# PM25/Information-Retrieval-with-Contrastive-Learning

Hardware: AMD Instinct MI355X
Metric: query-doc pairs/sec (train) + queries/sec @ top-k over N docs, 1/2/4/8 GPU (higher is better)
Workload: dtype bf16

## Files before the change

include/irc.h:

```cpp
#ifndef IRC_H_
#define IRC_H_

#include <stdint.h>

#ifdef __cplusplus
extern "C" {
#endif

typedef void* irc_stream_t;

#define IRC_OK 0
#define IRC_E_INVALID 1001
#define IRC_E_WORKSPACE 1002
#define IRC_E_LAUNCH 1003

const char* irc_last_error(void);
int irc_abi_version(void);

int64_t irc_scan_topk_workspace(int64_t Q, int64_t N, int64_t D, int64_t k);
int irc_scan_topk(const void* queries, const void* docs, int64_t Q, int64_t N, int64_t D,
                  int64_t k, int64_t doc_offset, void* workspace, int64_t workspace_bytes,
                  float* out_score, int64_t* out_idx, irc_stream_t stream);

int irc_scan_topk_many(const void* const* queries, int64_t batches, const void* docs, int64_t Q,
// ... 57 lines not shown
                      int64_t workspace_bytes, float* out_score, int64_t* out_idx,
                      irc_stream_t stream);
int irc_scan_scores_fp8(const void* queries, const void* docs, int64_t Q, int64_t N, int64_t D,
                        float* out, irc_stream_t stream);
int irc_quantize_fp8(int in_dtype, const void* x, int64_t n, float scale, void* out,
                     irc_stream_t stream);

int irc_gemm(int in_dtype, int out_dtype, int a_layout, int b_layout, int epilogue, int64_t M,
             int64_t N, int64_t K, float alpha, const void* A, int64_t lda, int64_t strideA,
             const void* B, int64_t ldb, int64_t strideB, const float* bias, int64_t strideBias,
             const void* R, int64_t ldr, int64_t strideR, void* C, int64_t ldc, int64_t strideC,
             int accumulate, int64_t batch, void* workspace, int64_t workspace_bytes,
             irc_stream_t stream);
int64_t irc_gemm_workspace(int in_dtype, int out_dtype, int epilogue, int64_t M, int64_t N,
                           int64_t K, int64_t batch);
int irc_gemm_ex(int in_dtype, int out_dtype, int a_layout, int b_layout, int epilogue, int64_t M,
                int64_t N, int64_t K, float alpha, const void* A, int64_t lda, int64_t strideA,
                const void* B, int64_t ldb, int64_t strideB, const float* bias, int64_t strideBias,
                const void* R, int64_t ldr, int64_t strideR, void* C, int64_t ldc, int64_t strideC,
                int accumulate, int64_t batch, void* workspace, int64_t workspace_bytes,
                int64_t max_blocks, irc_stream_t stream);
int64_t irc_gemm_workspace_ex(int in_dtype, int out_dtype, int epilogue, int64_t M, int64_t N,
                              int64_t K, int64_t batch, int64_t max_blocks);
int irc_gemm_set_persistent(int mode);
int irc_gemm_set_big_ring(int on);
int irc_gemm_ln(int epilogue, int64_t M, int64_t N, int64_t K, const void* A, int64_t lda,
                const void* B, int64_t ldb, const float* bias, const void* R, int64_t ldr,
                void* C, int64_t ldc, const float* ln_stats, int ln_nt, const float* ln_gamma,
                const float* ln_beta, float ln_eps, int64_t ln_h, const float* fold_colsum,
                float* stats_out, int* stats_nt_out, irc_stream_t stream);
int irc_gemm_set_big_mf16(int on);
int irc_gemm_set_big_dma(int on);
int irc_gemm_big_dma_fits(int64_t M, int64_t N, int64_t K, int64_t lda, int64_t ldb);

int irc_gemm_set_pp(int on);

int irc_embed_ln(int dtype, const int64_t* ids, const void* word, const void* pos,
                 const void* type0, const float* gamma, const float* beta, void* y, int64_t rows,
                 int64_t L, int64_t H, float eps, irc_stream_t stream);
int irc_layernorm(int dtype, const void* x, void* y, const float* gamma, const float* beta,
                  int64_t rows, int64_t H, float eps, irc_stream_t stream);
int irc_attention(int dtype, const void* qkv, const int64_t* mask, void* ctx, int64_t B,
                  int64_t L, int64_t H, int64_t heads, irc_stream_t stream);
int irc_qkv_attention(int64_t M, int64_t H, int64_t heads, int64_t L, const void* x, int64_t ldx,
                      const void* wqkv_perm, const float* bias_perm, const int64_t* mask,
                      void* ctx, int64_t ldc, irc_stream_t stream);

int64_t irc_layernorm_bwd_workspace(int64_t rows, int64_t H);
int irc_layernorm_bwd(int dtype, int dy_dtype, const void* dy, const void* x, const float* gamma,
                      void* dx, float* dgamma, float* dbeta, float* partial,
                      int64_t partial_floats, int64_t rows, int64_t H, float eps, int64_t bcast_L,
                      float dy_scale, int accumulate, irc_stream_t stream);
int irc_attention_bwd(int dtype, const void* qkv, const int64_t* mask, const void* ctx,
                      const void* dctx, void* dqkv, int64_t B, int64_t L, int64_t H,
                      int64_t heads, irc_stream_t stream);
int irc_embed_sum(int dtype, const int64_t* ids, const void* word, const void* pos,
                  const void* type0, float* y, int64_t rows, int64_t L, int64_t H,
                  irc_stream_t stream);
int irc_embed_bwd(int dtype, const void* dx, const int64_t* ids, float* dword, float* dpos,
                  float* dtype0, float* workspace, int64_t ws_floats, int64_t B, int64_t L,
                  int64_t H, int64_t pad_id, irc_stream_t stream);

int irc_lstm_fwd(int dtype, const float* xp, const void* whh, void* hout, float* gsave,
                 float* csave, void* hprev, int64_t B, int64_t L, int64_t H, int64_t ndir,
                 irc_stream_t stream);
int irc_lstm_bwd(int dtype, const float* dy, const void* whh, const float* gsave,
// ... 159 lines not shown
```

information-retrieval-with-contrastive-learning_amd/csrc/gemm.hip:

```cpp
#include "gemm_epi.h"
#include "gemm_pp.h"

#include <algorithm>
#include <atomic>
#include <type_traits>

#ifndef IRC_GEMM_GROUP_M
#define IRC_GEMM_GROUP_M 0
#endif

namespace irc {
namespace gemm {

enum Layout { ROW = 0, COL = 1 };

constexpr int BM = 128, BN = 128, NT = 256;

template <typename T>
struct TT;
template <>
struct TT<unsigned short> {
  static constexpr int BK = 32;
  static constexpr int VEC = 8;
  static constexpr int PITCH = BK * 2 + 16;
};
template <>
struct TT<float> {
  static constexpr int BK = 16;
  static constexpr int VEC = 4;
  static constexpr int PITCH = BK * 4 + 16;
};

struct Args {
  const void* A;
  const void* B;
  void* C;
  const float* bias;
  const void* R;
  int M, N, K;
  int64_t lda, ldb, ldc, ldr;
  int64_t sA, sB, sC, sR, sBias;
  float alpha;
  int accumulate;
  int vec_a, vec_b;
  int vec_c;
  int kchunk;
  float* P;
  int group_m;
  LnArgs ln;
  int big_dma;
};

__device__ __forceinline__ int kimg_off(int row, int ch) {
  return 256 * row + 16 * (ch ^ (((row & 3) << 2) | ((row >> 2) & 3)));
}
__device__ __forceinline__ bf16x8 kimg_frag(const char* img, int col0, int ks, int lane) {
  const int g = lane >> 4, j = lane & 15, q = j >> 2, p = j & 3;
  const int c = col0 + 16 * (g & 1);
  const int k0 = ks * 16 + 8 * (g >> 1);
  const int cb = c / 8 + (p >> 1), b8 = 8 * (p & 1);
  const v4s lo = ds_tr16(img + kimg_off(k0 + q, cb) + b8);
  const v4s hi = ds_tr16(img + kimg_off(k0 + 4 + q, cb) + b8);
  const v4s both[2] = {lo, hi};
  return __builtin_bit_cast(bf16x8, both);
}

template <typename T, int LAYOUT>
struct Slab {
  static constexpr int BK = TT<T>::BK;
  static constexpr int VEC = TT<T>::VEC;
  static constexpr int NVEC = (128 * BK) / VEC;
  static constexpr int PER_T = NVEC / NT;
  u16x8 v[PER_T];

  __device__ __forceinline__ void load(const T* base, int64_t ld, int row0, int nrows, int k0,
                                       int K, bool vec) {
    const int tid = threadIdx.x;
#pragma unroll
    for (int i = 0; i < PER_T; ++i) {
      const int e = i * NT + tid;
      int r, kk;
      if (LAYOUT == ROW) {
        r = e / (BK / VEC);
// ... 277 lines not shown
template <int ROWS>
__device__ __forceinline__ void stage(const unsigned short* __restrict__ X, int64_t ld, int r0,
                                      int nrows, int k0, char* lds_tile, int wave, int lane,
                                      int ls = 0, int sh = 6) {
  constexpr int PASSES = ROWS * 8 / NT;
#pragma unroll
  for (int i = 0; i < PASSES; ++i) {
    const int p = (i * NW + wave) * 64 + lane;
    const int row = p >> 3;
    const int c = (p & 7) ^ chunk_key(row);
    int gr = ls == 0 ? r0 + row
                     : ((r0 + row) >> sh) * ls + min(row & ((1 << sh) - 1), ls - 1);
    gr = gr < nrows ? gr : nrows - 1;
    glds16(X + (int64_t)gr * ld + k0 + c * 8, lds_tile + (i * NW + wave) * 1024);
  }
}
template <int ROWS>
__device__ __forceinline__ void stage_buf(__amdgpu_buffer_rsrc_t rsrc, uint32_t lane_off,
                                          uint32_t soff, uint32_t pass_bytes, char* lds_tile,
                                          int wave) {
  constexpr int PASSES = ROWS * 8 / NT;
#pragma unroll
  for (int i = 0; i < PASSES; ++i)
    blds16(rsrc, lane_off, soff + i * pass_bytes, lds_tile + (i * NW + wave) * 1024);
}
__device__ __forceinline__ uint32_t dma_lane_off(int64_t ld, int wave, int lane, int ls = 0) {
  const int row0 = 8 * wave + (lane >> 3);
  const int gr = ls == 0 ? row0 : min(row0, ls - 1);
  return (uint32_t)gr * (uint32_t)ld * 2u + (uint32_t)(((lane & 7) ^ chunk_key(row0)) * 16);
}
inline bool dma_fits(int64_t rows, int64_t K, int64_t ld) {
  if (rows <= 0 || K <= 0 || ld < 0 || ld > (1ll << 31)) return false;
  return ((rows - 1) * ld + K) * 2 < (1ll << 31);
}

constexpr int BK4 = 32, ROW4 = BK4 * 2, NST = 4;
template <int ROWS>
__device__ __forceinline__ void stage4(const unsigned short* __restrict__ X, int64_t ld, int r0,
                                       int nrows, int k0, char* lds_tile, int wave, int lane) {
  constexpr int CH = ROWS * 4;
  static_assert(CH % NT == 0, "whole passes");
#pragma unroll
  for (int i = 0; i < CH / NT; ++i) {
    const int p = (i * NW + wave) * 64 + lane;
    const int row = p >> 2;
    const int c = (p & 3) ^ ((row >> 2) & 3);
    int gr = r0 + row;
    gr = gr < nrows ? gr : nrows - 1;
    glds16(X + (int64_t)gr * ld + k0 + c * 8, lds_tile + (i * NW + wave) * 1024);
  }
}

#ifdef IRC_BIG_STAMPS
__device__ uint64_t big_stamps[64][5][2];
#define BSTAMP(kt, i)                                                                      \
  do {                                                                                     \
    __builtin_amdgcn_sched_barrier(0);                                                     \
    if (blockIdx.x == 0 && threadIdx.x == 0 && (kt) < 64) {                               \
      uint64_t c_, r_;                                                                     \
      asm volatile("s_memtime %0\n\ts_memrealtime %1\n\ts_waitcnt lgkmcnt(0)"            \
                   : "=s"(c_), "=s"(r_)::"memory");                                        \
      *(volatile uint64_t*)&big_stamps[(kt)][(i)][0] = c_;                                 \
      *(volatile uint64_t*)&big_stamps[(kt)][(i)][1] = r_;                                 \
    }                                                                                      \
    __builtin_amdgcn_sched_barrier(0);                                                     \
  } while (0)
#else
#define BSTAMP(kt, i) \
  do {                \
  } while (0)
#endif

template <int WNB>
__device__ __forceinline__ void mainloop_mf16(const unsigned short* A, int64_t lda,
                                              const unsigned short* B, int64_t ldb, int m0,
                                              int n0, int M, int N, int K, char* lds, int wave,
                                              int lane, f32x4 (&acc4)[8][2 * WNB], bool dma,
                                              int ls = 0, int sh = 6) {
  constexpr int BN = 128 * WNB;
  constexpr int A_BYTES = BM * ROW_BYTES, STAGE = A_BYTES + BN * ROW_BYTES;
  const int wm = wave >> 2, wn = wave & 3;
  const int nk = K / BK;
  const int a_rows = ls == 0 ? 64 : ls;
  const int a_row0 = ls == 0 ? m0 : (m0 >> sh) * ls;
  const bool buf = dma && (ls == 0 || sh == 6) && a_row0 + (BM / 64) * a_rows <= M && n0 + BN <= N;
  const __amdgpu_buffer_rsrc_t ra = buffer_rsrc(A, (uint32_t)(((int64_t)(M - 1) * lda + K) * 2));
  const __amdgpu_buffer_rsrc_t rb = buffer_rsrc(B, (uint32_t)(((int64_t)(N - 1) * ldb + K) * 2));
  const uint32_t a_pass = (uint32_t)a_rows * (uint32_t)lda * 2u, b_pass = 128u * (uint32_t)ldb;
  const uint32_t a_tile = (uint32_t)a_row0 * (uint32_t)lda * 2u;
  const uint32_t b_tile = (uint32_t)n0 * (uint32_t)ldb * 2u;
  uint32_t a_lane = 0, b_lane = 0;
  if (buf) {
    a_lane = dma_lane_off(lda, wave, lane, ls);
    b_lane = dma_lane_off(ldb, wave, lane);
    stage_buf<BM>(ra, a_lane, a_tile, a_pass, lds, wave);
    stage_buf<BN>(rb, b_lane, b_tile, b_pass, lds + A_BYTES, wave);
  } else {
    stage<BM>(A, lda, m0, M, 0, lds, wave, lane, ls, sh);
    stage<BN>(B, ldb, n0, N, 0, lds + A_BYTES, wave, lane);
  }
  wait_vmcnt<0>();
  __syncthreads();
  const int l16 = lane & 15, q4 = lane >> 4;
  const int key = chunk_key(l16);
  for (int kt = 0; kt < nk; ++kt) {
    const int cur = kt & 1;
#ifdef IRC_PP_DIAG_NODMA
    const bool more = kt + 1 < nk && kt < 0;
#else
    const bool more = kt + 1 < nk;
#endif
    BSTAMP(kt, 0);
    char* nxt = lds + (cur ^ 1) * STAGE;
    if (more && buf) {
      const uint32_t kb = (uint32_t)(kt + 1) * ROW_BYTES;
      stage_buf<BM>(ra, a_lane, a_tile + kb, a_pass, nxt, wave);
      stage_buf<BN>(rb, b_lane, b_tile + kb, b_pass, nxt + A_BYTES, wave);
    } else if (more) {
      int ln = lane;
      asm volatile("" : "+v"(ln));
      stage<BM>(A, lda, m0, M, (kt + 1) * BK, nxt, wave, ln, ls, sh);
      stage<BN>(B, ldb, n0, N, (kt + 1) * BK, nxt + A_BYTES, wave, ln);
    }
    BSTAMP(kt, 1);
    const char* la = lds + cur * STAGE;
    const char* lb = la + A_BYTES;
#pragma unroll
    for (int s2 = 0; s2 < 2; ++s2) {
      const int coff = (((4 * s2 + q4) ^ key) * 16);
      bf16x8 fa[8];
#pragma unroll
      for (int i = 0; i < 8; ++i)
        fa[i] = *reinterpret_cast<const bf16x8*>(la + (wm * 128 + i * 16 + l16) * 128 + coff);
#pragma unroll
      for (int j = 0; j < 2 * WNB; ++j) {
        const bf16x8 fb =
            *reinterpret_cast<const bf16x8*>(lb + (wn * 32 * WNB + j * 16 + l16) * 128 + coff);
#pragma unroll
        for (int i = 0; i < 8; ++i)
          acc4[i][j] = __builtin_amdgcn_mfma_f32_16x16x32_bf16(fa[i], fb, acc4[i][j], 0, 0, 0);
      }
    }
    BSTAMP(kt, 2);
    wait_vmcnt<0>();
    BSTAMP(kt, 3);
    __syncthreads();
    BSTAMP(kt, 4);
  }
}
}

inline std::atomic<int>& big_ring_mode() {
  static std::atomic<int> on{0};
  return on;
}
inline bool big_ring() { return big_ring_mode().load(std::memory_order_relaxed) != 0; }

inline std::atomic<int>& big_mf16_mode() {
  static std::atomic<int> on{1};
  return on;
}
inline bool big_mf16() { return big_mf16_mode().load(std::memory_order_relaxed) != 0; }

inline std::atomic<int>& big_dma_mode() {
  static std::atomic<int> on{1};
  return on;
}
inline int big_dma_flag(int64_t M, int64_t N, int64_t K, int64_t lda, int64_t ldb) {
  return big_dma_mode().load(std::memory_order_relaxed) != 0 && big::dma_fits(M, K, lda) &&
         big::dma_fits(N, K, ldb);
}

template <int EPI, int WNB>
__device__ __forceinline__ void big_epilogue_bf16(const Args& g, const f32x4 (&acc4)[8][2 * WNB],
                                                  char* lds, unsigned short* C,
                                                  const unsigned short* R, const float* bias,
                                                  int m0, int n0, int wave, int lane) {
  constexpr int BN = 128 * WNB, WCOLS = 32 * WNB, PITCH = WCOLS + 8;
  constexpr int CPR = WCOLS / 8;
  constexpr int NCH = 32 * CPR / 64;
  constexpr int NB = CPR == 12 ? 3 : 1;
  constexpr int RSTEP = 64 * NB / CPR;
  static_assert(64 * NB % CPR == 0 && NCH % NB == 0, "the chunk map repeats every NB iterations");
  constexpr bool READS_R = EPI == EPI_BIAS_RESID || EPI == EPI_RESID || EPI == EPI_DGELU;
  constexpr bool USES_R = READS_R || EPI == EPI_BIAS_GELU_SAVE;
  const int wm = wave >> 2, wn = wave & 3;
  float* st = reinterpret_cast<float*>(lds) + wave * (32 * PITCH);
  const int rbase0 = m0 + wm * 128;
  const int cbase = n0 + wn * WCOLS;
  const bool fast = m0 + big::BM <= g.M && n0 + BN <= g.N && g.ldc < (1 << 24) &&
                    (!USES_R || g.ldr < (1 << 24));
  float bv[2 * WNB];
#pragma unroll
  for (int j = 0; j < 2 * WNB; ++j) {
    const int col = cbase + j * 16 + (lane & 15);
    bv[j] = epi_has_bias(EPI) && col < g.N ? bias[col] : 0.f;
  }
  const f32x2_t alpha = {g.alpha, g.alpha};
  float* sw = st + 4 * (lane >> 4) * PITCH + (lane & 15);

  auto finish = [&](const f32x4& v0, const f32x4& v1, const u16x8& rr,
                    const unsigned short* rp) -> u16x8 {
    float v[8] = {v0[0], v0[1], v0[2], v0[3], v1[0], v1[1], v1[2], v1[3]};
// ... 171 lines not shown
    for (int kt = 0; kt < nk; ++kt) {
      const int after = nk - 1 - kt;
      if (after >= 2) wait_vmcnt<2 * PPT>();
      else if (after == 1) wait_vmcnt<PPT>();
      else wait_vmcnt<0>();
      wg_barrier();
      if (kt + 3 < nk) {
        char* nxt = lds + ((kt + 3) & 3) * STG4;
        big::stage4<BM>(A, g.lda, m0, g.M, (kt + 3) * BK4, nxt, wave, lane);
        big::stage4<BN>(B, g.ldb, n0, g.N, (kt + 3) * BK4, nxt + A4, wave, lane);
      }
      const char* la = lds + (kt & 3) * STG4;
      const char* lb = la + A4;
#pragma unroll
      for (int kk = 0; kk < BK4 / 16; ++kk) {
        const int coff = ((2 * kk + h) ^ sw4) * 16;
        bf16x8 fa[4], fb[WNB];
#pragma unroll
        for (int i = 0; i < 4; ++i)
          fa[i] = *reinterpret_cast<const bf16x8*>(la + (wm * 128 + i * 32 + r32) * ROW4 + coff);
#pragma unroll
        for (int j = 0; j < WNB; ++j)
          fb[j] = *reinterpret_cast<const bf16x8*>(lb + (wn * 32 * WNB + j * 32 + r32) * ROW4 + coff);
#pragma unroll
        for (int i = 0; i < 4; ++i)
#pragma unroll
          for (int j = 0; j < WNB; ++j)
            acc[i][j] = __builtin_amdgcn_mfma_f32_32x32x16_bf16(fa[i], fb[j], acc[i][j], 0, 0, 0);
      }
    }
    __syncthreads();
  } else if constexpr (MF16) {
    big::mainloop_mf16<WNB>(A, g.lda, B, g.ldb, m0, n0, g.M, g.N, g.K, lds, wave, lane, acc4,
                            g.big_dma != 0);
  } else {
  const int nk = g.K / BK;
  big::stage<BM>(A, g.lda, m0, g.M, 0, lds, wave, lane);
  big::stage<BN>(B, g.ldb, n0, g.N, 0, lds + A_BYTES, wave, lane);
  wait_vmcnt<0>();
  __syncthreads();
  const int swz = big::chunk_key(r32);
  for (int kt = 0; kt < nk; ++kt) {
    const int cur = kt & 1;
#ifdef IRC_PP_DIAG_NODMA
    const bool more = kt + 1 < nk && kt < 0;
#else
    const bool more = kt + 1 < nk;
#endif
    if (more) {
      char* nxt = lds + (cur ^ 1) * STAGE;
      big::stage<BM>(A, g.lda, m0, g.M, (kt + 1) * BK, nxt, wave, lane);
      big::stage<BN>(B, g.ldb, n0, g.N, (kt + 1) * BK, nxt + A_BYTES, wave, lane);
    }
    const char* la = lds + cur * STAGE;
    const char* lb = la + A_BYTES;
#pragma unroll
    for (int kk = 0; kk < BK / 16; ++kk) {
      const int coff = (((2 * kk + h) ^ swz) * 16);
      bf16x8 fa[4], fb[WNB];
#pragma unroll
      for (int i = 0; i < 4; ++i)
        fa[i] = *reinterpret_cast<const bf16x8*>(la + (wm * 128 + i * 32 + r32) * 128 + coff);
#pragma unroll
      for (int j = 0; j < WNB; ++j)
        fb[j] = *reinterpret_cast<const bf16x8*>(lb + (wn * 32 * WNB + j * 32 + r32) * 128 + coff);
#pragma unroll
      for (int i = 0; i < 4; ++i)
// ... 238 lines not shown
          if constexpr (sizeof(TO) == 2)
            r = bf16_to_f32(reinterpret_cast<const unsigned short*>(R)[(int64_t)row * g.ldr + col]);
          else
            r = reinterpret_cast<const float*>(R)[(int64_t)row * g.ldr + col];
          v = EPI == EPI_DGELU ? v * gelu_grad_fast(r) : v + r;
        }
        TO* dst = C + (int64_t)row * g.ldc + col;
        if constexpr (sizeof(TO) == 2) {
          *reinterpret_cast<unsigned short*>(dst) = f32_to_bf16(v);
        } else {
          if (g.accumulate)
            *reinterpret_cast<float*>(dst) += v;
          else
            *reinterpret_cast<float*>(dst) = v;
        }
      }
    }
  }
}

typedef __bf16 bf16x2_v __attribute__((ext_vector_type(2)));
struct QaArgs {
  const unsigned short* x;
  const unsigned short* w;
  const float* bias;
  const int64_t* mask;
  unsigned short* ctx;
  int M, K, H;
  int64_t ldx, ldc;
  float scale;
  int L;
  int group_m;
  int big_dma;
};

template <int SL>
__global__ __launch_bounds__(big::NT, 1) void qkv_attn_kernel(QaArgs g) {
  constexpr bool PACK = SL == 0;
  constexpr int WNB = 3, BM = big::BM, BN = 128 * WNB, TP = BN + 8;
  constexpr int SLX = PACK ? 128 : SL;
  constexpr int SH = SLX == 64 ? 6 : 7;
  constexpr int NJM = SLX / 32;
  __shared__ __attribute__((aligned(1024))) char lds[2 * (BM + BN) * big::ROW_BYTES];
  static_assert(128 * TP * 2 + 8 * SLX * 4 <= 2 * (BM + BN) * big::ROW_BYTES,
                "staged half and mask biases fit the LDS");
  const int nseq = g.M / g.L;
  const int spt = PACK ? BM / g.L : BM / SLX;
  const int ls = PACK || g.L == SL ? 0 : g.L;
  const int tiles_m = (nseq + spt - 1) / spt;
  const int tiles_n = 3 * g.H / BN;
  const int ntiles = tiles_m * tiles_n;
  int bid = blockIdx.x;
  {
    const int q = ntiles / 8, r = ntiles % 8, x = bid % 8;
    bid = (x < r ? x * (q + 1) : r * (q + 1) + (x - r) * q) + bid / 8;
  }
  int tm, tn;
  grouped_tile(bid, tiles_m, tiles_n, g.group_m, tm, tn);
  const int m0 = PACK ? tm * spt * g.L : tm * BM, n0 = tn * BN;
  const int lane = threadIdx.x & 63;
  const int wave = __builtin_amdgcn_readfirstlane(threadIdx.x >> 6);
  const int wm = wave >> 2, wn = wave & 3;
  f32x4 acc4[8][2 * WNB];
#pragma unroll
  for (int i = 0; i < 8; ++i)
#pragma unroll
    for (int j = 0; j < 2 * WNB; ++j) acc4[i][j] = (f32x4)0.0f;
  big::mainloop_mf16<WNB>(g.x, g.ldx, g.w, g.K, m0, n0, g.M, 3 * g.H, g.K, lds, wave, lane, acc4,
                          g.big_dma != 0, ls, SH);

  unsigned short* T = reinterpret_cast<unsigned short*>(lds);
  float* mbw = reinterpret_cast<float*>(lds + 128 * TP * 2) + SL * wave;
  uint32_t pk[8][2 * WNB][2];
#pragma unroll
  for (int j = 0; j < 2 * WNB; ++j) {
    const int col = n0 + wn * 32 * WNB + 16 * j + (lane & 15);
    const float bvj = g.bias[col];
#pragma unroll
    for (int i = 0; i < 8; ++i)
#pragma unroll
      for (int e2 = 0; e2 < 2; ++e2) {
        f32x2_t v;
#pragma unroll
        for (int u = 0; u < 2; ++u) v[u] = acc4[i][j][2 * e2 + u] * 1.0f + bvj;
        uint32_t w = __builtin_bit_cast(uint32_t, __builtin_convertvector(v, bf16x2_v));
        asm volatile("" : "+v"(w));
        pk[i][j][e2] = w;
      }
  }
  const int h = lane >> 5, r32 = lane & 31;
  const int nj = (g.L + 31) / 32;
  if constexpr (PACK) {
    constexpr int TQ = 264;
    static_assert(BM * TQ * 2 + 8 * 128 * 4 <= 2 * (BM + BN) * big::ROW_BYTES,
                  "staged head and mask biases fit the LDS");
    unsigned short* Tq = reinterpret_cast<unsigned short*>(lds);
    float* mb = reinterpret_cast<float*>(lds + BM * TQ * 2) + 128 * wave;
    const int odd = lane & 1;
    const uint32_t psel = odd ? 0x03020706u : 0x05040100u;
    const int nsq = min(spt, nseq - tm * spt);
    const int nit = nsq * nj;
#pragma unroll
// ... 215 lines not shown
              const v4s hi = ds_tr16(reinterpret_cast<const char*>(vp + 8 * TP));
              const v4s both[2] = {lo, hi};
              o[db] = __builtin_amdgcn_mfma_f32_32x32x16_bf16(pa, __builtin_bit_cast(bf16x8, both),
                                                              o[db], 0, 0, 0);
            }
          }
        }
#pragma unroll
        for (int db = 0; db < 2; ++db)
#pragma unroll
          for (int e = 0; e < 16; ++e) {
            const int i = 32 * ib + (e & 3) + 8 * (e >> 2) + 4 * h;
            if (i < g.L) out[(int64_t)i * g.ldc + 32 * db + r32] = f32_to_bf16(o[db][e]);
          }
      }
    }
    if (hf == 0) __syncthreads();
  }
}

inline int big_wnb(const Args& g, int batch, int la, int lb) {
  if (la != ROW || lb != ROW || !g.vec_a || !g.vec_b) return 0;
  if (g.K % big::BK != 0 || g.K == 0) return 0;
  const int wnb = g.N % 384 == 0 ? 3 : 2;
  const int64_t tiles = (int64_t)((g.M + 255) / 256) * ((g.N + 128 * wnb - 1) / (128 * wnb)) * batch;
  return tiles >= 128 ? wnb : 0;
}

template <typename TO, int EPI, bool LN = false>
static int launch_big(const Args& g0, int batch, int wnb, hipStream_t st) {
  Args g = g0;
  g.big_dma = big_dma_flag(g.M, g.N, g.K, g.lda, g.ldb);
  const int bn = 128 * wnb;
  const int tiles = ((g.M + big::BM - 1) / big::BM) * ((g.N + bn - 1) / bn);
  prof_begin(st);
  const bool ring = big_ring() && g.K % big::BK4 == 0;
  if constexpr (LN) {
    if (wnb == 3)
      hipLaunchKernelGGL((gemm_big_kernel<TO, EPI, 3, false, true, true>), dim3(tiles, batch), dim3(big::NT), 0, st, g);
    else
      hipLaunchKernelGGL((gemm_big_kernel<TO, EPI, 2, false, true, true>), dim3(tiles, batch), dim3(big::NT), 0, st, g);
  } else if (big_mf16() && !ring) {
    if (wnb == 3)
      hipLaunchKernelGGL((gemm_big_kernel<TO, EPI, 3, false, true>), dim3(tiles, batch), dim3(big::NT), 0, st, g);
    else
      hipLaunchKernelGGL((gemm_big_kernel<TO, EPI, 2, false, true>), dim3(tiles, batch), dim3(big::NT), 0, st, g);
  } else if (wnb == 3 && ring)
    hipLaunchKernelGGL((gemm_big_kernel<TO, EPI, 3, true>), dim3(tiles, batch), dim3(big::NT), 0, st, g);
  else if (wnb == 3)
    hipLaunchKernelGGL((gemm_big_kernel<TO, EPI, 3>), dim3(tiles, batch), dim3(big::NT), 0, st, g);
  else if (ring)
    hipLaunchKernelGGL((gemm_big_kernel<TO, EPI, 2, true>), dim3(tiles, batch), dim3(big::NT), 0, st, g);
  else
    hipLaunchKernelGGL((gemm_big_kernel<TO, EPI, 2>), dim3(tiles, batch), dim3(big::NT), 0, st, g);
  prof_end("gemm_bf16", st, 2.0 * g.M * g.N * g.K * batch);
  prof_work("gemm_bf16_bytes", gemm_alg_bytes(sizeof(TO) == 4, EPI, g.accumulate, g.M, g.N, g.K,
                                               batch));
  return check_launch("gemm_big_kernel");
}

template <typename TI, typename TO, int LA, int LB, int EPI>
static int launch(const Args& g0, int batch, int splits, hipStream_t st) {
  if constexpr (sizeof(TI) == 2) {
    if (splits == 1) {
      const int wnb = big_wnb(g0, batch, LA, LB);
      if (wnb) return launch_big<TO, EPI>(g0, batch, wnb, st);
// ... 132 lines not shown
    ln.nt_out = (int)((N + 255) / 256);
    pa.ln = ln;
    if (stats_nt_out) *stats_nt_out = ln.nt_out;
    prof_begin(st);
    gpp::run_ln(epilogue, pa, st);
    prof_end("gemm_bf16", st, flops);
    prof_work("gemm_bf16_bytes", gemm_alg_bytes(0, epilogue, 0, M, N, K, 1));
    return check_launch("gemm_pp_kernel(ln)");
  }
  ln.nt_out = (int)((N + 128 * wnb - 1) / (128 * wnb));
  g.ln = ln;
  if (stats_nt_out) *stats_nt_out = ln.nt_out;
  switch (epilogue) {
    case EPI_BIAS: return launch_big<unsigned short, EPI_BIAS, true>(g, 1, wnb, st);
    case EPI_BIAS_GELU: return launch_big<unsigned short, EPI_BIAS_GELU, true>(g, 1, wnb, st);
    default: return launch_big<unsigned short, EPI_BIAS_RESID, true>(g, 1, wnb, st);
  }
}

extern "C" int irc_qkv_attention(int64_t M, int64_t H, int64_t heads, int64_t L, const void* x,
                                 int64_t ldx, const void* wqkv_perm, const float* bias_perm,
                                 const int64_t* mask, void* ctx, int64_t ldc,
                                 irc_stream_t stream) {
  using namespace irc::gemm;
  IRC_REQUIRE(L >= 1 && L <= 128 && heads * 64 == H && H % 128 == 0,
              "qkv_attention: needs L <= 128, head dim 64 and H %% 128 == 0");
  IRC_REQUIRE(M > 0 && M % L == 0 && M < (1ll << 31), "qkv_attention: M must be a multiple of L");
  IRC_REQUIRE(H % 64 == 0 && ldx % 8 == 0 && ldx >= H && ldc >= H, "qkv_attention: bad strides");
  IRC_REQUIRE((((uintptr_t)x | (uintptr_t)wqkv_perm) % 16) == 0 && ((uintptr_t)ctx % 2) == 0,
              "qkv_attention: operands must be 16-byte aligned");
  IRC_REQUIRE(bias_perm != nullptr, "qkv_attention: bias required");
  QaArgs a{static_cast<const unsigned short*>(x), static_cast<const unsigned short*>(wqkv_perm),
           bias_perm, mask, static_cast<unsigned short*>(ctx), (int)M, (int)H, (int)H, ldx, ldc,
           0.125f, (int)L, IRC_GEMM_GROUP_M, big_dma_flag(M, 3 * H, H, ldx, H)};
  hipStream_t st = as_stream(stream);
  const int64_t nseq = M / L, tiles_n = 3 * H / 384;
  const int slot = L <= 64 ? 4 : 2;
  const int64_t ncu = std::max(1, gpp::cu_count() > 0 ? gpp::cu_count() : 256);
  const auto waves = [&](int64_t s) { return ((nseq + s - 1) / s * tiles_n + ncu - 1) / ncu; };
  const bool packed = 256 / L > slot && waves(256 / L) < waves(slot);
  const int spt = packed ? (int)(256 / L) : slot;
  const int tiles = (int)(((nseq + spt - 1) / spt) * tiles_n);
  prof_begin(st);
  if (packed)
    hipLaunchKernelGGL(qkv_attn_kernel<0>, dim3(tiles), dim3(big::NT), 0, st, a);
  else if (L <= 64)
    hipLaunchKernelGGL(qkv_attn_kernel<64>, dim3(tiles), dim3(big::NT), 0, st, a);
  else
    hipLaunchKernelGGL(qkv_attn_kernel<128>, dim3(tiles), dim3(big::NT), 0, st, a);
  prof_end("gemm_bf16", st, 2.0 * M * 3 * H * H);
  prof_work("gemm_bf16_bytes", 2.0 * (double)M * H + 2.0 * 3 * H * H + 2.0 * (double)M * H);
  return check_launch("qkv_attn_kernel");
}

#ifdef IRC_BIG_STAMPS
extern "C" int irc_big_dbg_stamps(uint64_t* out ) {
  if (hipDeviceSynchronize() != hipSuccess) return -1;
  return hipMemcpyFromSymbol(out, HIP_SYMBOL(irc::gemm::big::big_stamps),
                             sizeof(irc::gemm::big::big_stamps)) == hipSuccess ? 0 : -1;
}
#endif

extern "C" int irc_gemm_set_big_mf16(int on) {
  return irc::gemm::big_mf16_mode().exchange(on ? 1 : 0);
}

extern "C" int irc_gemm_set_big_dma(int on) {
  return irc::gemm::big_dma_mode().exchange(on ? 1 : 0);
}

extern "C" int irc_gemm_big_dma_fits(int64_t M, int64_t N, int64_t K, int64_t lda, int64_t ldb) {
  return irc::gemm::big::dma_fits(M, K, lda) && irc::gemm::big::dma_fits(N, K, ldb) ? 1 : 0;
}

extern "C" int irc_gemm_set_big_ring(int on) {
  return irc::gemm::big_ring_mode().exchange(on ? 1 : 0);
}

extern "C" int irc_gemm_ex(int in_dtype, int out_dtype, int a_layout, int b_layout, int epilogue,
                           int64_t M, int64_t N, int64_t K, float alpha, const void* A, int64_t lda,
                           int64_t strideA, const void* B, int64_t ldb, int64_t strideB,
                           const float* bias, int64_t strideBias, const void* R, int64_t ldr,
                           int64_t strideR, void* C, int64_t ldc, int64_t strideC, int accumulate,
                           int64_t batch, void* workspace, int64_t workspace_bytes,
                           int64_t max_blocks, irc_stream_t stream) {
  const int64_t bud = split_budget(max_blocks);
  IRC_REQUIRE(M >= 0 && N >= 0 && K >= 0 && batch >= 1, "gemm: bad sizes");
  IRC_REQUIRE(M < (1ll << 31) && N < (1ll << 31) && K < (1ll << 31), "gemm: size too large");
  IRC_REQUIRE(in_dtype == 0 || in_dtype == 1, "gemm: in_dtype must be 0 (bf16) or 1 (fp32)");
  IRC_REQUIRE(out_dtype == 0 || out_dtype == 1, "gemm: out_dtype must be 0 (bf16) or 1 (fp32)");
  IRC_REQUIRE(!(accumulate && out_dtype == 0), "gemm: accumulate needs fp32 C");
  IRC_REQUIRE(epilogue >= 0 && epilogue <= 6, "gemm: bad epilogue");
  IRC_REQUIRE(!gemm::epi_has_bias(epilogue) || bias, "gemm: epilogue needs bias");
  IRC_REQUIRE(!(epilogue >= 3 && epilogue != 1 && epilogue != 2) || R,
              "gemm: epilogue needs R (residual / pre-activation)");
  IRC_REQUIRE(!(accumulate && epilogue >= 5), "gemm: accumulate with a GELU epilogue");
  const int vec = in_dtype == 0 ? 8 : 4;
  const int vec_a = lda % vec == 0 && strideA % vec == 0 && ((uintptr_t)A % 16) == 0;
  const int vec_b = ldb % vec == 0 && strideB % vec == 0 && ((uintptr_t)B % 16) == 0;
  if (M == 0 || N == 0) return IRC_OK;
  int splits = gemm::split_count(in_dtype == 0 ? 2 : 4, out_dtype == 1, epilogue, M, N, K, batch, bud);
  if (splits > 1 && (workspace == nullptr ||
                     workspace_bytes < (int64_t)splits * M * N * batch * (int64_t)sizeof(float)))
    splits = 1;
  const int cvec = out_dtype == 0 ? 8 : 4;
// ... 59 lines not shown
```

information-retrieval-with-contrastive-learning_amd/irc_amd/_lib.py:

```python
from __future__ import annotations

import ctypes
import os
import threading

_HERE = os.path.dirname(os.path.abspath(__file__))
LIB_PATH = os.path.join(_HERE, "lib", "libirc_hip.so")
LIB_PATH = os.environ.get("IRC_LIB_PATH") or LIB_PATH

_c = ctypes
P = _c.c_void_p
I64 = _c.c_int64
I32 = _c.c_int
U32 = _c.c_uint32
F32 = _c.c_float

SIGNATURES = {
    "irc_last_error": (_c.c_char_p, []),
    "irc_abi_version": (I32, []),
    "irc_scan_topk_workspace": (I64, [I64, I64, I64, I64]),
    "irc_scan_topk": (I32, [P, P, I64, I64, I64, I64, I64, P, I64, P, P, P]),
    "irc_scan_topk_many": (I32, [P, I64, P, I64, I64, I64, I64, I64, P, I64, I64, P, P, P, P]),
    "irc_corpus_pack": (I32, [P, P, I64, I64, P, P, P]),
    "irc_pair_sample": (I32, [P, P, P, P, I64, P, P]),
# ... 13 lines not shown
    "irc_rerank_topk_fp8": (I32, [P, P, I64, I64, I64, P, P, I64, I64, I64, F32, P, I64, P, P, P,
                                  P]),
    "irc_rerank_topk_stream_fp8": (I32, [P, P, I64, I64, I64, P, P, I64, I64, I64, F32, P, I64, P,
                                         P, P, P]),
    "irc_rerank_topk_grouped_workspace": (I64, [I64, I64, I64]),
    "irc_rerank_topk_grouped": (I32, [P, P, I64, I64, I64, P, P, I64, I64, I64, P, I64, U32, F32,
                                      P, I64, P, P, P, P]),
    "irc_scan_topk_fp8_workspace": (I64, [I64, I64, I64, I64]),
    "irc_scan_topk_fp8": (I32, [P, P, I64, I64, I64, I64, I64, F32, P, I64, P, P, P]),
    "irc_scan_scores_fp8": (I32, [P, P, I64, I64, I64, P, P]),
    "irc_quantize_fp8": (I32, [I32, P, I64, F32, P, P]),
    "irc_csr_union_chunks": (I64, [I64]),
    "irc_csr_union_count": (I32, [P, P, I64, P, P, I64, I64, P, P, P]),
    "irc_csr_union_emit": (I32, [P, I64, I64, P, P, P, P]),
    "irc_csr_spmv_f64": (I32, [P, P, P, I64, P, P, P, I64, P, P]),
    "irc_topk_f64": (I32, [P, I64, P, P, I64, I64, P, P, P, P]),
    "irc_proto_ce": (I32, [P, P, I64, I64, P, P, P, P]),
    "irc_argmax_bias": (I32, [P, P, I64, I64, P, P, P]),
    "irc_centroid_accumulate": (I32, [P, P, I64, I64, P, P, P]),
    "irc_centroid_finalize": (I32, [P, P, I64, I64, P, P, P]),
    "irc_gemm": (I32, [I32, I32, I32, I32, I32, I64, I64, I64, F32, P, I64, I64, P, I64, I64,
                       P, I64, P, I64, I64, P, I64, I64, I32, I64, P, I64, P]),
    "irc_gemm_workspace": (I64, [I32, I32, I32, I64, I64, I64, I64]),
    "irc_gemm_ex": (I32, [I32, I32, I32, I32, I32, I64, I64, I64, F32, P, I64, I64, P, I64, I64,
                          P, I64, P, I64, I64, P, I64, I64, I32, I64, P, I64, I64, P]),
    "irc_gemm_workspace_ex": (I64, [I32, I32, I32, I64, I64, I64, I64, I64]),
    "irc_gemm_set_persistent": (I32, [I32]),
    "irc_gemm_set_big_ring": (I32, [I32]),
    "irc_gemm_ln": (I32, [I32, I64, I64, I64, P, I64, P, I64, P, P, I64, P, I64, P, I32, P, P, F32,
                          I64, P, P, P, P]),
    "irc_gemm_set_big_mf16": (I32, [I32]),
    "irc_gemm_set_big_dma": (I32, [I32]),
    "irc_gemm_big_dma_fits": (I32, [I64, I64, I64, I64, I64]),
    "irc_gemm_set_pp": (I32, [I32]),
    "irc_scan_set_ppl_min_q": (I32, [I32]),
    "irc_embed_ln": (I32, [I32, P, P, P, P, P, P, P, I64, I64, I64, F32, P]),
    "irc_layernorm": (I32, [I32, P, P, P, P, I64, I64, F32, P]),
    "irc_attention": (I32, [I32, P, P, P, I64, I64, I64, I64, P]),
    "irc_qkv_attention": (I32, [I64, I64, I64, I64, P, I64, P, P, P, P, I64, P]),
    "irc_layernorm_bwd_workspace": (I64, [I64, I64]),
    "irc_layernorm_bwd": (I32, [I32, I32, P, P, P, P, P, P, P, I64, I64, I64, F32, I64, F32, I32,
                                P]),
    "irc_attention_bwd": (I32, [I32, P, P, P, P, P, I64, I64, I64, I64, P]),
    "irc_embed_sum": (I32, [I32, P, P, P, P, P, I64, I64, I64, P]),
    "irc_embed_bwd": (I32, [I32, P, P, P, P, P, P, I64, I64, I64, I64, I64, P]),
    "irc_lstm_fwd": (I32, [I32, P, P, P, P, P, P, I64, I64, I64, I64, P]),
    "irc_lstm_bwd": (I32, [I32, P, P, P, P, P, I64, I64, I64, I64, P]),
    "irc_lstm_mfma_supported": (I32, [I64]),
    "irc_lstm_mfma_save_floats": (I64, [I64, I64, I64, I64, I32]),
    "irc_lstm_pack": (I32, [P, P, P, P, I64, I64, I64, P, P, P, P, P]),
    "irc_lstm_fwd_mfma": (I32, [P, P, P, P, P, P, I64, I64, I64, I64, P]),
    "irc_lstm_bwd_mfma": (I32, [P, P, P, P, P, I64, I64, I64, I64, P]),
    "irc_lstm_hprev": (I32, [P, P, I64, I64, I64, I64, P]),
    "irc_lstm_coop_supported": (I32, [I64]),
    "irc_lstm_coop_sizes": (I64, [I64, I64, I64, I64, I32]),
    "irc_lstm_coop_pack": (I32, [P, I64, I64, P, P, P]),
    "irc_lstm_fwd_coop": (I32, [P, P, P, P, P, P, P, P, I64, I64, I64, I64, P]),
    "irc_lstm_bwd_coop": (I32, [P, P, P, P, P, P, P, I64, I64, I64, I64, P]),
    "irc_lstm_coop_fault": (I32, [P, I64, I64, P, P]),
    "irc_mean_rows": (I32, [I32, P, P, I64, I64, I64, I64, P]),
    "irc_bcast_rows": (I32, [P, P, I64, I64, I64, F32, P]),
    "irc_l2norm_fwd": (I32, [P, P, P, I64, I64, F32, P]),
    "irc_l2norm_bwd": (I32, [P, P, P, P, I64, I64, F32, P]),
    "irc_nce_lse": (I32, [P, P, I64, I64, F32, P, P, P]),
    "irc_nce_grads": (I32, [P, P, P, I64, I64, F32, P, P, P, P]),
    "irc_axpby": (I32, [P, P, P, F32, F32, I64, P]),
# ... 76 lines not shown
```

information-retrieval-with-contrastive-learning_amd/irc_amd/ops.py:

```python
from __future__ import annotations

import ctypes

import torch

from . import _lib
from ._lib import IRCError
from ._torch import ptr, require_hip, stream_ptr

BF16, F32 = torch.bfloat16, torch.float32
_DT = {BF16: 0, F32: 1}

EPI_NONE, EPI_BIAS, EPI_BIAS_GELU, EPI_BIAS_RESID, EPI_RESID = 0, 1, 2, 3, 4


def _code(t: torch.Tensor) -> int:
    try:
        return _DT[t.dtype]
    except KeyError:
        raise TypeError(f"irc kernels take bf16 or fp32, got {t.dtype}") from None


def gemm_set_big_ring(on) -> int:
    return int(_lib.load().irc_gemm_set_big_ring(1 if on else 0))
# ... 27 lines not shown
            raise ValueError(f"gemm_ln: {name} has {t.numel()} elements, needs {n}")
    if stats is not None and (stats.t.shape[0] != M or stats.h != (N if residual is not None else K)):
        raise ValueError("gemm_ln: the statistics describe another activation")
    if out is None:
        out = torch.empty((M, N), dtype=BF16, device=a.device)
    st_out = None
    if want_stats:
        st_out = torch.empty((M, (N + 127) // 128, 2), dtype=F32, device=a.device)
    nt = ctypes.c_int(0)
    _lib.call("irc_gemm_ln", int(epilogue), M, N, K, ptr(a), a.stride(0), ptr(b), b.stride(0),
              ptr(bias), ptr(residual), residual.stride(0) if residual is not None else 0,
              ptr(out), out.stride(0), ptr(stats.t) if stats is not None else None,
              stats.nt if stats is not None else 0, ptr(gamma), ptr(beta), float(eps),
              stats.h if stats is not None else 0, ptr(colsum), ptr(st_out),
              ctypes.addressof(nt) if want_stats else None, stream_ptr(a.device))
    if want_stats:
        n = int(nt.value)
        return out, LnStats(st_out.view(-1)[:M * n * 2].view(M, n, 2), n, N)
    return out


def gemm_set_big_mf16(on) -> int:
    return int(_lib.load().irc_gemm_set_big_mf16(1 if on else 0))


def gemm_set_big_dma(on) -> int:
    return int(_lib.load().irc_gemm_set_big_dma(1 if on else 0))


def gemm_big_dma_fits(M, N, K, lda, ldb) -> bool:
    return bool(_lib.load().irc_gemm_big_dma_fits(M, N, K, lda, ldb))


def gemm_set_pp(on) -> int:
    return int(_lib.load().irc_gemm_set_pp(1 if on else 0))


def gemm_set_persistent(mode) -> int:
    return int(_lib.load().irc_gemm_set_persistent(int(mode)))


def gemm(a, b, *, trans_a=False, b_is_nk=True, bias=None, epilogue=EPI_NONE, residual=None,
         alpha=1.0, out=None, out_dtype=None, accumulate=False, max_blocks=0):
    require_hip(a, b, bias, residual, out)
    if a.dtype != b.dtype:
        raise TypeError(f"gemm operands must share a dtype ({a.dtype} vs {b.dtype})")
    if a.stride(-1) != 1 or b.stride(-1) != 1:
        raise ValueError("gemm operands must be contiguous in their last dim")
    M, K = (a.shape[1], a.shape[0]) if trans_a else (a.shape[0], a.shape[1])
    N, Kb = (b.shape[0], b.shape[1]) if b_is_nk else (b.shape[1], b.shape[0])
    if K != Kb:
        raise ValueError(f"gemm inner dims differ: {K} vs {Kb}")
    if out is None:
        od = out_dtype or a.dtype
        out = torch.empty((M, N), dtype=od, device=a.device)
        if accumulate:
            out.zero_()
    if bias is not None and bias.dtype != F32:
        raise TypeError("bias must be fp32")
    if residual is not None and residual.dtype != out.dtype:
        raise TypeError("residual dtype must match the output")
    ws, nws = _splitk_ws(a, out, epilogue, M, N, K, 1, max_blocks)
    _lib.call("irc_gemm_ex", _code(a), _code(out), 1 if trans_a else 0, 0 if b_is_nk else 1,
              int(epilogue), M, N, K, float(alpha), ptr(a), a.stride(0), 0, ptr(b), b.stride(0),
              0, ptr(bias), 0, ptr(residual), residual.stride(0) if residual is not None else 0, 0,
              ptr(out), out.stride(0), 0, 1 if accumulate else 0, 1, ptr(ws), nws,
# ... 564 lines not shown
```

Before: 34630.

## Add cooperative L2 prefetch touches to big GEMM DMA mainloop

Adds an L2 prefetch scheme to the mf16 buffer-DMA GEMM mainloop. Tiles that share A or B rows within a concurrency window each issue masked single-dword loads for a disjoint slice of rows TOUCH_D k-steps ahead, so the shared operand lines get pulled into L2 once, ahead of use. It is on by default (mode 1) when big_dma is active, group_m<=1 and tiles_n<=2, and it also covers the fused QKV-attention path. It costs extra load instructions and vmcnt pressure in the hot loop, and the prefetch may duplicate traffic that L2 would already serve.

New measurement: 35000, median of 6. 1.1% higher.

```diff
diff --git a/include/irc.h b/include/irc.h
--- a/include/irc.h
+++ b/include/irc.h
@@ -113,6 +113,10 @@
 int irc_gemm_set_big_mf16(int on);
 int irc_gemm_set_big_dma(int on);
 int irc_gemm_big_dma_fits(int64_t M, int64_t N, int64_t K, int64_t lda, int64_t ldb);
+int irc_gemm_set_l2_touch(int mode);
+int64_t irc_gemm_l2_touch_map(int operand, int64_t tiles_m, int64_t tiles_n, int64_t window,
+                              int64_t lines, int64_t nk, int64_t dist, int32_t* count,
+                              int32_t* owner, int32_t* sharers);
 
 int irc_gemm_set_pp(int on);
 
diff --git a/information-retrieval-with-contrastive-learning_amd/csrc/gemm.hip b/information-retrieval-with-contrastive-learning_amd/csrc/gemm.hip
--- a/information-retrieval-with-contrastive-learning_amd/csrc/gemm.hip
+++ b/information-retrieval-with-contrastive-learning_amd/csrc/gemm.hip
@@ -49,6 +49,7 @@
   int group_m;
   LnArgs ln;
   int big_dma;
+  int l2_touch;
 };
 
 __device__ __forceinline__ int kimg_off(int row, int ch) {
@@ -392,6 +393,54 @@
 inline bool dma_fits(int64_t rows, int64_t K, int64_t ld) {
   if (rows <= 0 || K <= 0 || ld < 0 || ld > (1ll << 31)) return false;
   return ((rows - 1) * ld + K) * 2 < (1ll << 31);
+}
+
+#ifndef IRC_BIG_TOUCH_D
+#define IRC_BIG_TOUCH_D 2
+#endif
+constexpr int TOUCH_D = IRC_BIG_TOUCH_D;
+struct Touch {
+  int a_lo, a_n, b_lo, b_n;
+};
+__host__ __device__ inline void touch_share(int tiles_m, int tiles_n, int window, int tm, int tn,
+                                            int& s_a, int& rank_a, int& s_b, int& rank_b) {
+  s_a = tiles_n < window ? tiles_n : window;
+  s_a = s_a < 1 ? 1 : s_a;
+  rank_a = tn % s_a;
+  s_b = window / (tiles_n < 1 ? 1 : tiles_n);
+  s_b = s_b > tiles_m ? tiles_m : s_b;
+  s_b = s_b < 1 ? 1 : s_b;
+  rank_b = tm % s_b;
+}
+__host__ __device__ inline void touch_range(int lines, int s, int rank, int& lo, int& n) {
+  lo = rank * lines / s;
+  n = (rank + 1) * lines / s - lo;
+}
+__host__ __device__ inline Touch touch_lines(int window, int tiles_m, int tiles_n, int tm, int tn,
+                                             int a_lines, int b_lines) {
+  Touch t{0, 0, 0, 0};
+  if (window <= 0) return t;
+  int s_a, rank_a, s_b, rank_b;
+  touch_share(tiles_m, tiles_n, window, tm, tn, s_a, rank_a, s_b, rank_b);
+  touch_range(a_lines, s_a, rank_a, t.a_lo, t.a_n);
+  touch_range(b_lines, s_b, rank_b, t.b_lo, t.b_n);
+  return t;
+}
+__device__ __forceinline__ void touch_dword(uint32_t& sink, __amdgpu_buffer_rsrc_t rsrc,
+                                            uint32_t voff, uint32_t soff, uint64_t mask) {
+#ifdef __HIP_DEVICE_COMPILE__
+  asm volatile(
+      "s_mov_b64 exec, %1\n\t"
+      "buffer_load_dword %0, %2, %3, %4 offen\n\t"
+      "s_mov_b64 exec, -1"
+      : "+v"(sink)
+      : "s"(mask), "v"(voff), "s"(rsrc), "s"(soff));
+#endif
+}
+__device__ __forceinline__ void touch_done(uint32_t sink) {
+#ifdef __HIP_DEVICE_COMPILE__
+  asm volatile("" ::"v"(sink));
+#endif
 }
 
 constexpr int BK4 = 32, ROW4 = BK4 * 2, NST = 4;
@@ -436,7 +485,7 @@
                                               const unsigned short* B, int64_t ldb, int m0,
                                               int n0, int M, int N, int K, char* lds, int wave,
                                               int lane, f32x4 (&acc4)[8][2 * WNB], bool dma,
-                                              int ls = 0, int sh = 6) {
+                                              const Touch tch, int ls = 0, int sh = 6) {
   constexpr int BN = 128 * WNB;
   constexpr int A_BYTES = BM * ROW_BYTES, STAGE = A_BYTES + BN * ROW_BYTES;
   const int wm = wave >> 2, wn = wave & 3;
@@ -450,6 +499,19 @@
   const uint32_t a_tile = (uint32_t)a_row0 * (uint32_t)lda * 2u;
   const uint32_t b_tile = (uint32_t)n0 * (uint32_t)ldb * 2u;
   uint32_t a_lane = 0, b_lane = 0;
+  uint32_t ta_lane = 0, tb_lane = 0, sink = 0;
+  uint64_t ta_mask = 0, tb_mask = 0;
+  int touch_nk = 0;
+  if (buf && (tch.a_n | tch.b_n) != 0) {
+    touch_nk = nk - TOUCH_D;
+    const int t = wave * 64 + lane;
+    const int ar = tch.a_lo + t;
+    const int arow = ls == 0 ? ar : (ar >> 6) * ls + min(ar & 63, ls - 1);
+    ta_lane = (uint32_t)arow * (uint32_t)lda * 2u;
+    tb_lane = (uint32_t)(tch.b_lo + t) * (uint32_t)ldb * 2u;
+    ta_mask = __builtin_amdgcn_ballot_w64(t < tch.a_n);
+    tb_mask = __builtin_amdgcn_ballot_w64(t < tch.b_n);
+  }
   if (buf) {
     a_lane = dma_lane_off(lda, wave, lane, ls);
     b_lane = dma_lane_off(ldb, wave, lane);
@@ -476,6 +538,11 @@
       const uint32_t kb = (uint32_t)(kt + 1) * ROW_BYTES;
       stage_buf<BM>(ra, a_lane, a_tile + kb, a_pass, nxt, wave);
       stage_buf<BN>(rb, b_lane, b_tile + kb, b_pass, nxt + A_BYTES, wave);
+      if (kt < touch_nk) {
+        const uint32_t kd = (uint32_t)(kt + TOUCH_D) * ROW_BYTES;
+        if (ta_mask != 0) touch_dword(sink, ra, ta_lane, a_tile + kd, ta_mask);
+        if (tb_mask != 0) touch_dword(sink, rb, tb_lane, b_tile + kd, tb_mask);
+      }
     } else if (more) {
       int ln = lane;
       asm volatile("" : "+v"(ln));
@@ -507,6 +574,7 @@
     __syncthreads();
     BSTAMP(kt, 4);
   }
+  touch_done(sink);
 }
 }
 
@@ -529,6 +597,22 @@
 inline int big_dma_flag(int64_t M, int64_t N, int64_t K, int64_t lda, int64_t ldb) {
   return big_dma_mode().load(std::memory_order_relaxed) != 0 && big::dma_fits(M, K, lda) &&
          big::dma_fits(N, K, ldb);
+}
+
+constexpr int L2_TOUCH_MAX_TILES_N = 2;
+inline std::atomic<int>& l2_touch_mode() {
+  static std::atomic<int> mode{[] {
+    const char* e = getenv("IRC_GEMM_L2_TOUCH");
+    return e && e[0] >= '0' && e[0] <= '2' ? e[0] - '0' : 1;
+  }()};
+  return mode;
+}
+inline int l2_touch_flag(int big_dma, int group_m, int64_t tiles_n) {
+  const int mode = l2_touch_mode().load(std::memory_order_relaxed);
+  if (mode == 0 || !big_dma || group_m > 1) return 0;
+  if (mode == 1 && tiles_n > L2_TOUCH_MAX_TILES_N) return 0;
+  const int cus = gpp::cu_count();
+  return cus >= 8 ? cus / 8 : 32;
 }
 
 template <int EPI, int WNB>
@@ -766,7 +850,8 @@
     __syncthreads();
   } else if constexpr (MF16) {
     big::mainloop_mf16<WNB>(A, g.lda, B, g.ldb, m0, n0, g.M, g.N, g.K, lds, wave, lane, acc4,
-                            g.big_dma != 0);
+                            g.big_dma != 0,
+                            big::touch_lines(g.l2_touch, tiles_m, tiles_n, tm, tn, BM, BN));
   } else {
   const int nk = g.K / BK;
   big::stage<BM>(A, g.lda, m0, g.M, 0, lds, wave, lane);
@@ -1071,6 +1156,7 @@
   int L;
   int group_m;
   int big_dma;
+  int l2_touch;
 };
 
 template <int SL>
@@ -1106,7 +1192,8 @@
 #pragma unroll
     for (int j = 0; j < 2 * WNB; ++j) acc4[i][j] = (f32x4)0.0f;
   big::mainloop_mf16<WNB>(g.x, g.ldx, g.w, g.K, m0, n0, g.M, 3 * g.H, g.K, lds, wave, lane, acc4,
-                          g.big_dma != 0, ls, SH);
+                          g.big_dma != 0,
+                          big::touch_lines(g.l2_touch, tiles_m, tiles_n, tm, tn, BM, BN), ls, SH);
 
   unsigned short* T = reinterpret_cast<unsigned short*>(lds);
   float* mbw = reinterpret_cast<float*>(lds + 128 * TP * 2) + SL * wave;
@@ -1388,6 +1475,7 @@
   Args g = g0;
   g.big_dma = big_dma_flag(g.M, g.N, g.K, g.lda, g.ldb);
   const int bn = 128 * wnb;
+  g.l2_touch = l2_touch_flag(g.big_dma, g.group_m, (g.N + bn - 1) / bn);
   const int tiles = ((g.M + big::BM - 1) / big::BM) * ((g.N + bn - 1) / bn);
   prof_begin(st);
   const bool ring = big_ring() && g.K % big::BK4 == 0;
@@ -1586,7 +1674,8 @@
   IRC_REQUIRE(bias_perm != nullptr, "qkv_attention: bias required");
   QaArgs a{static_cast<const unsigned short*>(x), static_cast<const unsigned short*>(wqkv_perm),
            bias_perm, mask, static_cast<unsigned short*>(ctx), (int)M, (int)H, (int)H, ldx, ldc,
-           0.125f, (int)L, IRC_GEMM_GROUP_M, big_dma_flag(M, 3 * H, H, ldx, H)};
+           0.125f, (int)L, IRC_GEMM_GROUP_M, big_dma_flag(M, 3 * H, H, ldx, H), 0};
+  a.l2_touch = l2_touch_flag(a.big_dma, a.group_m, 3 * H / 384);
   hipStream_t st = as_stream(stream);
   const int64_t nseq = M / L, tiles_n = 3 * H / 384;
   const int slot = L <= 64 ? 4 : 2;
@@ -1625,6 +1714,45 @@
 
 extern "C" int irc_gemm_big_dma_fits(int64_t M, int64_t N, int64_t K, int64_t lda, int64_t ldb) {
   return irc::gemm::big::dma_fits(M, K, lda) && irc::gemm::big::dma_fits(N, K, ldb) ? 1 : 0;
+}
+
+extern "C" int irc_gemm_set_l2_touch(int mode) {
+  return irc::gemm::l2_touch_mode().exchange(mode < 0 ? 0 : mode > 2 ? 2 : mode);
+}
+
+extern "C" int64_t irc_gemm_l2_touch_map(int operand, int64_t tiles_m, int64_t tiles_n,
+                                         int64_t window, int64_t lines, int64_t nk,
+                                         int64_t dist, int32_t* count, int32_t* owner,
+                                         int32_t* sharers) {
+  using namespace irc::gemm;
+  if ((operand != 0 && operand != 1) || tiles_m < 1 || tiles_n < 1 || window < 1 || lines < 1 ||
+      lines > big::NT || nk < 1 || dist < 1 || tiles_m > (1 << 20) || tiles_n > (1 << 20) ||
+      window > (1 << 20) || !count || !owner)
+    return -1;
+  for (int64_t i = 0; i < nk * lines; ++i) count[i] = 0, owner[i] = -1;
+  int s_a, rank_a, s_b, rank_b;
+  big::touch_share((int)tiles_m, (int)tiles_n, (int)window, 0, 0, s_a, rank_a, s_b, rank_b);
+  const int s = operand == 0 ? s_a : s_b;
+  if (sharers) *sharers = s;
+  int64_t outside = 0;
+  for (int rank = 0; rank < s; ++rank) {
+    const big::Touch t = big::touch_lines((int)window, (int)tiles_m, (int)tiles_n,
+                                          operand == 0 ? 0 : rank, operand == 0 ? rank : 0,
+                                          (int)lines, (int)lines);
+    const int lo = operand == 0 ? t.a_lo : t.b_lo, n = operand == 0 ? t.a_n : t.b_n;
+    for (int64_t kt = 0; kt + dist < nk; ++kt)
+      for (int th = 0; th < big::NT; ++th) {
+        if (th >= n) continue;
+        const int64_t k = kt + dist, r = lo + th;
+        if (r < 0 || r >= lines || k >= nk) {
+          ++outside;
+          continue;
+        }
+        ++count[k * lines + r];
+        owner[k * lines + r] = rank;
+      }
+  }
+  return outside;
 }
 
 extern "C" int irc_gemm_set_big_ring(int on) {
diff --git a/information-retrieval-with-contrastive-learning_amd/irc_amd/_lib.py b/information-retrieval-with-contrastive-learning_amd/irc_amd/_lib.py
--- a/information-retrieval-with-contrastive-learning_amd/irc_amd/_lib.py
+++ b/information-retrieval-with-contrastive-learning_amd/irc_amd/_lib.py
@@ -69,6 +69,8 @@
     "irc_gemm_set_big_mf16": (I32, [I32]),
     "irc_gemm_set_big_dma": (I32, [I32]),
     "irc_gemm_big_dma_fits": (I32, [I64, I64, I64, I64, I64]),
+    "irc_gemm_set_l2_touch": (I32, [I32]),
+    "irc_gemm_l2_touch_map": (I64, [I32, I64, I64, I64, I64, I64, I64, P, P, P]),
     "irc_gemm_set_pp": (I32, [I32]),
     "irc_scan_set_ppl_min_q": (I32, [I32]),
     "irc_embed_ln": (I32, [I32, P, P, P, P, P, P, P, I64, I64, I64, F32, P]),
diff --git a/information-retrieval-with-contrastive-learning_amd/irc_amd/ops.py b/information-retrieval-with-contrastive-learning_amd/irc_amd/ops.py
--- a/information-retrieval-with-contrastive-learning_amd/irc_amd/ops.py
+++ b/information-retrieval-with-contrastive-learning_amd/irc_amd/ops.py
@@ -83,6 +83,24 @@
     return bool(_lib.load().irc_gemm_big_dma_fits(M, N, K, lda, ldb))
 
 
+def gemm_set_l2_touch(mode) -> int:
+    return int(_lib.load().irc_gemm_set_l2_touch(int(mode)))
+
+
+def gemm_l2_touch_map(operand, tiles_m, tiles_n, window, lines, nk, dist):
+    import numpy as np
+
+    count = np.empty((nk, lines), dtype=np.int32)
+    owner = np.empty((nk, lines), dtype=np.int32)
+    sharers = ctypes.c_int(0)
+    outside = _lib.load().irc_gemm_l2_touch_map(
+        int(operand), tiles_m, tiles_n, window, lines, nk, dist, count.ctypes.data,
+        owner.ctypes.data, ctypes.addressof(sharers))
+    if outside < 0:
+        raise ValueError("gemm_l2_touch_map: bad arguments")
+    return count, owner, int(sharers.value), int(outside)
+
+
 def gemm_set_pp(on) -> int:
     return int(_lib.load().irc_gemm_set_pp(1 if on else 0))
 
```
